# fumiama/Retrieval-based-Voice-Conversion-WebUI

Measured on AMD Instinct MI355X. Metric: real-time factor (audio-sec/wall-sec), 48 kHz v2, 10 s clips, retrieval + NSF-HiFi-GAN decode, higher is better.
Workload: dtype fp16 MFMA operands + fp16 inter-stage streams (ResBlock outputs, ups output of stages 1-3), fp32 accumulate / in-block residual; fp32 MFMA prefilter + fp64 verified IVF distances; 1 GPU; BASELINE configs[1]: v2/48k, 1 x 10 s clip(s) per GPU, T=1198 frames, 599 queries/clip, IVF 10000x768 nlist=256 nprobe=1 k=8 index_rate=0.75; hipgraph=True, index_blob_bytes=32376576, launcher=single process

## Files before the change

retrieval-based-voice-conversion-webui_amd/csrc/ivf.hip:

```cpp
#include <algorithm>
#include <atomic>
#include <cfloat>
#include <cmath>
#include <cstdio>
#include <memory>
#include <string>
#include <vector>

#include "common.hpp"
#include "ivf_format.hpp"
#include "ivf_kmeans.hpp"
#include "ivf_kernels.hpp"
#include "ivf_lm_kernels.hpp"
#include "ivf_add_kernels.hpp"

using namespace rvcmi;

struct rvcmi_ivf {
    int device = 0;
    BlobHeader hdr;
    char* blob = nullptr;
    bool owns_blob = false;
    int64_t cap_nq = 0;
    int cap_nprobe = 0;
// ... 137 lines not shown
    float* feats;
    float rate, omr;
};
static bool search(rvcmi_ivf* h, int64_t nq, const float* q, int k, float* D, int64_t* I, hipStream_t st,
                   const BlendFuse* bf = nullptr) {
    if (!h || nq < 0 || (nq && (!q || !D || !I))) RVCMI_FAIL(RVCMI_ERR_INVALID, "null argument");
    if (k < 1 || k > KMAX)
        RVCMI_FAIL(RVCMI_ERR_INVALID, "k=%d outside [1,%d]: the kernels keep at most %d neighbours per query (RVC asks for 8, "
                   "pipeline.py:126; legacy top-1 tools/cmd/infer-pm-index256.py:161)", k, KMAX, KMAX);
    if (nq == 0) return false;
    DeviceGuard dg(h->device);
    reserve(h, nq);
    const BlobHeader& b = h->hdr;
    const int d = b.d;
    const int np = (int)std::min<int64_t>(b.nprobe, b.nlist);
    HIP_CHECK(hipMemsetAsync(h->flag.p, 0, 4, st));
    const double cflops = 3.0 * (double)nq * b.nlist * d;
    if (np == 1 && !h->opt.on("IVF_COARSE_F64")) {
        h->prof.launch("ivf_coarse", 2.0 * (double)nq * b.nlist * d, (double)nq * d * 4 + (double)b.nlist * d * 4 + 2.0 * nq * b.nlist * 4, st, [&] {
            if (h->cap_chunk <= 0 || !h->cscore.p) RVCMI_FAIL(RVCMI_ERR_INVALID, "coarse score scratch not reserved");
            for (int64_t qs = 0; qs < nq; qs += h->cap_chunk) {
                const int64_t nqc = std::min<int64_t>(h->cap_chunk, nq - qs);
                const int64_t big_blocks = ((b.nlist + 127) / 128) * ((nqc + 63) / 64);
                if (big_blocks >= 512) {
                    dim3 grid((unsigned)((b.nlist + 127) / 128), (unsigned)((nqc + 63) / 64));
                    hipLaunchKernelGGL((k_coarse_gemm<2, 4>), grid, dim3(256), 0, st, q + qs * d, h->centroids(), h->cnorm(), nqc,
                                       b.nlist, d, h->cscore.as<float>());
                } else {
                    dim3 grid((unsigned)((b.nlist + 31) / 32), (unsigned)((nqc + 31) / 32));
                    hipLaunchKernelGGL(k_coarse_gemm_ks, grid, dim3(256), 0, st, q + qs * d, h->centroids(), h->cnorm(), nqc,
                                       b.nlist, d, h->cscore.as<float>());
                }
                hipLaunchKernelGGL(k_coarse_pick, dim3((unsigned)((nqc + 3) / 4)), dim3(256), 0, st, q + qs * d, h->centroids(),
                                   h->cscore.as<float>(), nqc, b.nlist, d, b.cmax, h->assign.as<int64_t>() + qs);
            }
        });
    } else if (np == 1) {
        const size_t smem = align_up((size_t)QT * d * 4, 16) + 4 * QT * 16;
        h->prof.launch("ivf_coarse", cflops, (double)nq * d * 4 + (double)b.nlist * d * 4, st, [&] {
            hipLaunchKernelGGL(k_coarse1, dim3((unsigned)((nq + QT - 1) / QT)), dim3(256), smem, st, q, h->centroids_t(), nq,
                               b.nlist, d, h->assign.as<int64_t>());
        });
    } else {
        h->prof.launch("ivf_coarse", cflops, (double)nq * b.nlist * 8, st, [&] {
            const int64_t tot = nq * b.nlist;
            hipLaunchKernelGGL(k_coarse_dist, dim3((unsigned)((tot + 255) / 256)), dim3(256), 0, st, q, h->centroids(), nq,
                               b.nlist, d, h->cdist.as<double>());
            hipLaunchKernelGGL(k_coarse_select, dim3((unsigned)nq), dim3(64), 0, st, h->cdist.as<double>(), b.nlist, np,
                               h->assign.as<int64_t>());
        });
    }
    const bool lm_wanted = h->opt.geti("IVF_LM", 1) && !h->opt.on("IVF_GENERIC");
    if (lm_wanted && nq >= 64 && !h->lm_warned) {
        const char* why = lm_unusable_reason(h, nq);
        if (why) {
            h->lm_warned = true;
            fprintf(stderr, "[rvcmi] ivf search: %lld queries run on the query-major scan (every probed list is re-read per query) because the "
                    "list-major kernels do not take this call: %s.  Printed once per index.\n", (long long)nq, why);
        }
    }
    if (lm_wanted && lm_usable(h, nq) && h->lm_S.p && nq <= h->lm_cap_nq && h->lm_buf_nq > 0) {
        const int pitch = (int)align_up((uint64_t)h->lm_maxlen, 32);
// ... 452 lines not shown
```

retrieval-based-voice-conversion-webui_amd/csrc/ivf_kernels.hpp:

```cpp
#pragma once
#include <hip/hip_runtime.h>

#include <cfloat>
#include <cmath>
#include <cstdint>

#include "glue_kernels.hpp"
#include "ivf_format.hpp"

namespace rvcmi {


constexpr int QT = 4;

__global__ void __launch_bounds__(256) k_coarse1(const float* __restrict__ q, const float4* __restrict__ cent_t,
                                                 int64_t nq, int64_t nlist, int d, int64_t* __restrict__ assign) {
    extern __shared__ __attribute__((aligned(16))) char smem_raw[];
    float* qs = (float*)smem_raw;
    double* bd = (double*)(smem_raw + align_up((size_t)QT * d * 4, 16));
    int64_t* bi = (int64_t*)(bd + 4 * QT);
    const int64_t q0 = (int64_t)blockIdx.x * QT;
    const int nqb = (int)min((int64_t)QT, nq - q0);
    for (int i = threadIdx.x; i < QT * d; i += 256) {
        int qi = i / d;
        qs[i] = qi < nqb ? q[(q0 + qi) * d + (i - qi * d)] : 0.f;
    }
    __syncthreads();
    double best[QT];
    int64_t besti[QT];
#pragma unroll
    for (int k = 0; k < QT; ++k) { best[k] = INFINITY; besti[k] = INT64_MAX; }
    const int d4 = d >> 2;
// ... 39 lines not shown
        int64_t biv = bi[k];
        for (int w = 1; w < 4; ++w) {
            double od = bd[w * QT + k];
            int64_t oi = bi[w * QT + k];
            if (od < bdv || (od == bdv && oi < biv)) { bdv = od; biv = oi; }
        }
        assign[q0 + k] = biv;
    }
}

constexpr int CG_K = 32, CG_S = 33;
using f32x16 = __attribute__((ext_vector_type(16))) float;
template <int MQ, int NWC>
__global__ void __launch_bounds__(64 * NWC) k_coarse_gemm(const float* __restrict__ q, const float* __restrict__ cent,
                                                          const float* __restrict__ cn, int64_t nq, int64_t nlist, int d,
                                                          float* __restrict__ S) {
    constexpr int NT = 64 * NWC, QR = 32 * MQ, CR = 32 * NWC;
    __shared__ float Qs[QR * CG_S];
    __shared__ float Cs[CR * CG_S];
    const int64_t q0 = (int64_t)blockIdx.y * QR, c0 = (int64_t)blockIdx.x * CR;
    const int wave = threadIdx.x >> 6, lane = threadIdx.x & 63;
    f32x16 acc[MQ];
#pragma unroll
    for (int m = 0; m < MQ; ++m)
#pragma unroll
        for (int e = 0; e < 16; ++e) acc[m][e] = 0.f;
    constexpr int SLOTS = (QR + CR) * (CG_K / 4);
    static_assert(SLOTS % NT == 0, "staging slots must divide evenly");
    constexpr int PER = SLOTS / NT;
    float4 pre[PER];
    auto fetch = [&](int k0) {
#pragma unroll
// ... 62 lines not shown
            float* dst = st + (idx >> 3) * CG_S + (idx & 7) * 4;
            const float4 v = pre[c % D][s2];
            dst[0] = v.x; dst[1] = v.y; dst[2] = v.z; dst[3] = v.w;
        }
        if (c + D < NCH) {
#pragma unroll
            for (int s2 = 0; s2 < 8; ++s2) pre[c % D][s2] = *(const float4*)(src[s2] + kw + (c + D) * kstep + coff);
        }
#pragma unroll
        for (int ks = 0; ks < CG_K / 2; ++ks) acc = __builtin_amdgcn_mfma_f32_32x32x2f32(qa[2 * ks], cb[2 * ks], acc, 0, 0, 0);
    }
}

__global__ void __launch_bounds__(256) k_coarse_gemm_ks(const float* __restrict__ q, const float* __restrict__ cent,
                                                        const float* __restrict__ cn, int64_t nq, int64_t nlist, int d,
                                                        float* __restrict__ S) {
    __shared__ float St[4][64 * CG_S];
    __shared__ float Red[3][64 * 16];
    const int64_t q0 = (int64_t)blockIdx.y * 32, c0 = (int64_t)blockIdx.x * 32;
    const int wave = threadIdx.x >> 6, lane = threadIdx.x & 63;
    float* st = St[wave];
    f32x16 acc;
#pragma unroll
    for (int e = 0; e < 16; ++e) acc[e] = 0.f;
    float4 pre[8];
    auto fetch = [&](int k0) {
#pragma unroll
        for (int it = 0; it < 8; ++it) {
            const int idx = lane + it * 64;
            const int row = idx >> 3, c4 = idx & 7;
            const int kk = min(k0 + c4 * 4, d - 4);
// ... 116 lines not shown
                a0 = fma(t0, t0, a0);
                a1 = fma(t1, t1, a1);
            }
            for (int off = 32; off >= 1; off >>= 1) {
                a0 += __shfl_xor(a0, off, 64);
                a1 += __shfl_xor(a1, off, 64);
            }
            if (a0 < best || (a0 == best && c0 + b0 < besti)) { best = a0; besti = c0 + b0; }
            if (two && (a1 < best || (a1 == best && c0 + b1 < besti))) { best = a1; besti = c0 + b1; }
        }
    }
    if (lane == 0) assign[qi] = besti;
}

__global__ void __launch_bounds__(256) k_coarse_dist(const float* __restrict__ q, const float* __restrict__ cent,
                                                     int64_t nq, int64_t nlist, int d, double* __restrict__ dist) {
    const int64_t i = (int64_t)blockIdx.x * 256 + threadIdx.x;
    if (i >= nq * nlist) return;
    const int64_t qi = i / nlist, c = i - qi * nlist;
    const float* a = q + qi * d;
    const float* b = cent + c * d;
    double acc = 0.0;
    for (int e = 0; e < d; ++e) {
        double t = (double)a[e] - (double)b[e];
        acc = fma(t, t, acc);
    }
    dist[i] = acc;
}
__global__ void __launch_bounds__(64) k_coarse_select(double* __restrict__ dist, int64_t nlist, int nprobe,
                                                      int64_t* __restrict__ assign) {
    const int64_t qi = blockIdx.x;
// ... 413 lines not shown
```

retrieval-based-voice-conversion-webui_amd/csrc/nsf.hip:

```cpp
#include <algorithm>
#include <atomic>
#include <cmath>
#include <functional>
#include <memory>
#include <string>
#include <unordered_map>

#include "common.hpp"
#include "nsf_kernels.hpp"
#include "conv_pack.hpp"
#include "rb_stream.hpp"

namespace rvcmi {

struct Geom {
    int MI, NJ, WCO, TT;
};
static Geom conv_geom(int cout) {
    Geom g;
    g.NJ = 4;
    if (cout >= 256) { g.MI = 2; g.WCO = 4; }
    else if (cout >= 128) { g.MI = 2; g.WCO = 2; }
    else if (cout >= 64) { g.MI = 2; g.WCO = 1; }
    else { g.MI = 1; g.WCO = 1; }
// ... 28 lines not shown
    float lin_w = 1.f, lin_b = 0.f;
    std::vector<Stage> stages;
    DevBuf post_w;
    int c_last = 0;
    size_t S = 0;
    DevBuf P, X0, Ya[RVCMI_MAX_RB], Yb[RVCMI_MAX_RB], H, NZ, har, har2, x2, phase, condv, dbg;
    size_t ws_bytes = 0;
    Profiler prof;
    rvcmi::Options opt;
};

namespace rvcmi {


static void set_lds_limits();
constexpr int RB_KG = 4;
#ifndef RB256_NJ
#define RB256_NJ 4
#endif
static int rb_rows(int C) { return C == 256 ? 32 * RB256_NJ : RB_ROWS; }
constexpr int RB_SPLIT_MAX_ROWS = 1024;
constexpr int RB_SPLIT_MAX_ROWS_128 = 4096;

static void build_stage(Stage& s, const rvcmi_nsf_config* cfg, const WeightMap& wm, int i) {
    const int op = cfg->operand, C0 = cfg->upsample_initial_channel;
    s.cin = C0 >> i;
    s.cout = C0 >> (i + 1);
    s.u = cfg->upsample_rates[i];
    s.k = cfg->upsample_kernel_sizes[i];
    s.pad = (s.k - s.u) / 2;
// ... 83 lines not shown
}

static void nsf_create(const rvcmi_nsf_config* cfg, const rvcmi_tensor* weights, int n_weights, int device, int max_B,
                       int max_T, rvcmi_nsf** out) {
    if (!cfg || !out || (!weights && n_weights)) RVCMI_FAIL(RVCMI_ERR_INVALID, "null argument");
    if (cfg->n_ups < 1 || cfg->n_ups > RVCMI_MAX_UPS || cfg->n_resblock_kernels < 1 ||
        cfg->n_resblock_kernels > RVCMI_MAX_RB)
        RVCMI_FAIL(RVCMI_ERR_INVALID, "bad stage counts");
    if (cfg->operand < 0 || cfg->operand > 2) RVCMI_FAIL(RVCMI_ERR_INVALID, "bad operand type %d", cfg->operand);
    if (max_B < 1 || max_T < 1) RVCMI_FAIL(RVCMI_ERR_INVALID, "max_B/max_T must be positive");
    HIP_CHECK(hipSetDevice(device));
    set_lds_limits();
    rb_stream_prepare();

    std::unique_ptr<rvcmi_nsf> h(new rvcmi_nsf());
    h->opt.load_env({"RB_STREAM", "NO_RB_SPLIT", "POST_DMA", "POST_DBG", "RBF_PAD_TAP", "RBF32_TALL", "DBG", "Y_F16", "X0_F16", "X0_F16_NOSTREAM"});
    rb_stream_load_env(h->opt);
    h->cfg = *cfg;
    h->device = device;
    h->max_B = max_B;
    h->max_T = max_T;
    const int op = cfg->operand;
    WeightMap wm;
    for (int i = 0; i < n_weights; ++i) wm.m[weights[i].name] = &weights[i];

    const int C0 = cfg->upsample_initial_channel, inter = cfg->inter_channels;
    h->C0 = C0;
    {
        const rvcmi_tensor& w = wm.get("conv_pre.weight", {C0, inter, 7});
        const rvcmi_tensor& b = wm.get("conv_pre.bias", {C0});
        const float* wd = w.data;
// ... 32 lines not shown
        upload(h->post_w, wt);
    }
    if (h->c_last & 3) RVCMI_FAIL(RVCMI_ERR_INVALID, "last stage channel count %d", h->c_last);

    if (cfg->n_resblock_kernels > 3) RVCMI_FAIL(RVCMI_ERR_INVALID, "more than 3 resblock kernels per stage is unsupported");
    h->S = S * (size_t)max_B;
    const size_t fb = h->S * sizeof(float);
    h->P.alloc((size_t)max_B * max_T * C0 * sizeof(float));
    h->X0.alloc(fb);
    for (int j = 0; j < cfg->n_resblock_kernels; ++j) {
        h->Ya[j].alloc(fb);
        h->Yb[j].alloc(fb);
    }
    if (op == RVCMI_OPERAND_F32) h->H.alloc(fb);
    else h->H.alloc((size_t)3 * std::max(RB_SPLIT_MAX_ROWS * 256, RB_SPLIT_MAX_ROWS_128 * 128) * 2);
    {
        size_t nz = 0;
        long Ls = max_T;
        for (int i = 0; i < cfg->n_ups; ++i) {
            Ls *= cfg->upsample_rates[i];
            if (h->stages[i].nz_mfma) nz = std::max(nz, (size_t)Ls * h->stages[i].cout);
        }
        if (nz) h->NZ.alloc(nz * max_B * sizeof(float));
    }
    const size_t hb = (size_t)max_B * max_T * upp * sizeof(float);
    h->har.alloc(hb);
    h->har2.alloc(hb);
    h->x2.alloc((size_t)max_B * inter * max_T * sizeof(float));
    h->phase.alloc((size_t)max_B * max_T * sizeof(float));
    h->condv.alloc((size_t)max_B * C0 * sizeof(float));
    HIP_CHECK(hipMemset(h->condv.p, 0, h->condv.bytes));
    h->ws_bytes = (size_t)(1 + 2 * cfg->n_resblock_kernels + (op == RVCMI_OPERAND_F32 ? 1 : 0)) * fb + h->P.bytes + 2 * hb + h->x2.bytes + h->phase.bytes + h->condv.bytes;
    *out = h.release();
}


template <typename OpT, int CIN, int MI, int NJ, int WCO>
static void launch_inst(const ConvArgs& a, int B, hipStream_t st) {
    using TL = Tile<CIN>;
    constexpr int TT = (4 / WCO) * NJ * 32;
    const int co_blocks = (a.cout + 32 * MI * WCO - 1) / (32 * MI * WCO);
    dim3 grid((a.Lq + TT - 1) / TT, co_blocks * a.nphase, B);
    const size_t smem = (size_t)a.tile_rows * TL::STRIDE;
    if (smem > 160 * 1024) RVCMI_FAIL(RVCMI_ERR_INVALID, "LDS tile too large: %zu bytes (cin %d)", smem, CIN);
    hipLaunchKernelGGL((k_conv_mfma<OpT, CIN, MI, NJ, WCO>), grid, dim3(256), smem, st, a);
}

// ... 83 lines not shown
static void launch_rb_pair(int op, int C, const RbPairArgs& ra, int tiles, int nj, int B, int rows, hipStream_t st) {
    if (op == RVCMI_OPERAND_BF16) launch_rb_pair_t<__bf16>(C, ra, tiles, nj, B, rows, st);
    else launch_rb_pair_t<_Float16>(C, ra, tiles, nj, B, rows, st);
}
template <typename OpT>
static void set_lds_rb() {
#define RB_ATTR(C_, MI_, NW_)                                                                                   \
    HIP_CHECK(hipFuncSetAttribute(reinterpret_cast<const void*>(&k_rb_pair<OpT, C_, MI_, NW_, RB_KG>),           \
                                  hipFuncAttributeMaxDynamicSharedMemorySize, 160 * 1024));
    HIP_CHECK(hipFuncSetAttribute(reinterpret_cast<const void*>(&k_rb_pair<OpT, 256, 2, 4, RB_KG, RB256_NJ>),
                                  hipFuncAttributeMaxDynamicSharedMemorySize, 160 * 1024));
    RB_ATTR(128, 2, 2) RB_ATTR(64, 2, 1) RB_ATTR(32, 1, 1) RB_ATTR(16, 1, 1)
#undef RB_ATTR
}

template <typename OpT, int CIN, int MI, int WV>
static void launch_ups_inst(UpsArgs a, int nj, int B, hipStream_t st) {
    const int TQ = 32 * nj * (4 / WV);
    size_t smem = (size_t)a.tile_rows * Tile<CIN>::STRIDE + (a.nz_k1 ? (size_t)(TQ * a.u * a.ns + 16) * 2 : 0);
    if (a.bias_off && a.cout % 4 == 0 && (smem + 15) / 16 * 16 + (size_t)2 * a.cout * 4 <= 160 * 1024) {
        smem = (smem + 15) / 16 * 16;
        a.bias_off = (int)smem;
        smem += (size_t)2 * a.cout * 4;
    } else {
        a.bias_off = 0;
    }
    if (smem > 160 * 1024) RVCMI_FAIL(RVCMI_ERR_INVALID, "upsampler LDS tile too large (%zu B)", smem);
    const int per_block = WV * a.vpw;
    dim3 grid((a.Lin + TQ - 1) / TQ, (a.nvt + per_block - 1) / per_block, B);
    {
        const int esz = a.out_half ? 2 : 4;
        const size_t ot = (size_t)TQ * a.u * ((size_t)a.cout * esz + 16);
        smem = (smem + 15) / 16 * 16;
        if (a.out_tr && grid.y == 1 && (a.cout * esz) % 16 == 0 && smem + ot <= 52 * 1024) {
            a.out_tr_off = (int)smem;
            smem += ot;
        } else {
            a.out_tr = 0;
        }
    }
    if (a.out_tw_off && !a.out_tr && a.out_half && nj == 1 && MI == 2 && a.cout % 64 == 0) {
        smem = (smem + 15) / 16 * 16;
        a.out_tw_off = (int)smem;
        smem += (size_t)4 * 32 * (MI * 64 + 16);
    } else {
        a.out_tw_off = 0;
    }
    if (nj == 4) hipLaunchKernelGGL((k_ups<OpT, CIN, MI, WV, 4>), grid, dim3(256), smem, st, a);
    else if (nj == 2) hipLaunchKernelGGL((k_ups<OpT, CIN, MI, WV, 2>), grid, dim3(256), smem, st, a);
    else hipLaunchKernelGGL((k_ups<OpT, CIN, MI, WV, 1>), grid, dim3(256), smem, st, a);
}
#define RVCMI_UPS_CASES(X, OpT) \
    X(OpT, 512, 2) X(OpT, 256, 2) X(OpT, 128, 2) X(OpT, 64, 1) X(OpT, 32, 1)
template <typename OpT>
static void launch_ups_t(const UpsArgs& a, int wv, int nj, int B, hipStream_t st) {
#define X(OpT_, CIN_, MI_)                                                        \
    if (a.cin == CIN_) {                                                          \
        if (wv == 4) return launch_ups_inst<OpT_, CIN_, MI_, 4>(a, nj, B, st);    \
        if (wv == 2) return launch_ups_inst<OpT_, CIN_, MI_, 2>(a, nj, B, st);    \
        return launch_ups_inst<OpT_, CIN_, MI_, 1>(a, nj, B, st);                 \
    }
    RVCMI_UPS_CASES(X, OpT)
#undef X
    RVCMI_FAIL(RVCMI_ERR_INVALID, "unsupported upsampler C_in %d", a.cin);
}
template <typename OpT>
static void set_lds_ups() {
#define Y(OpT_, CIN_, MI_, WV_, NJ_)                                                                                    \
    HIP_CHECK(hipFuncSetAttribute(reinterpret_cast<const void*>(&k_ups<OpT_, CIN_, MI_, WV_, NJ_>),                      \
                                  hipFuncAttributeMaxDynamicSharedMemorySize, 160 * 1024));
#define X(OpT_, CIN_, MI_)                                                                                              \
    Y(OpT_, CIN_, MI_, 4, 4) Y(OpT_, CIN_, MI_, 4, 2) Y(OpT_, CIN_, MI_, 4, 1) Y(OpT_, CIN_, MI_, 2, 4) Y(OpT_, CIN_, MI_, 2, 2)   \
    Y(OpT_, CIN_, MI_, 2, 1) Y(OpT_, CIN_, MI_, 1, 4) Y(OpT_, CIN_, MI_, 1, 2) Y(OpT_, CIN_, MI_, 1, 1)
    RVCMI_UPS_CASES(X, OpT)
#undef Y
#undef X
}

#ifndef RBF32_NJ
#define RBF32_NJ 3
#define RBF32_OCC 2
#endif
template <int C> struct RbFullGeom;
#ifndef RBF64_NWV
#define RBF64_NWV 8
#endif
#if RBF64_NWV == 8
template <> struct RbFullGeom<64> { static constexpr int MI = 2, NJ = 2, KG = 4, OCC = 2, NWV = 8; };
#else
template <> struct RbFullGeom<64> { static constexpr int MI = 2, NJ = 3, KG = 4, OCC = 1, NWV = 4; };
#endif
// ... 509 lines not shown
        ua.ph_w_off[r] = U.pack_off[r];
        ua.ph_in_off[r] = U.in_off[r];
        lo = std::min(lo, U.in_off[r] - (U.ntaps_p - 1));
        hi = std::max(hi, U.in_off[r]);
    }
    ua.ntaps_p = U.ntaps_p;
    ua.u = s.u;
    ua.cout = C;
    ua.lo = lo;
    ua.bias = U.bias.as<float>();
    ua.out = h->X0.as<float>();
    ua.out_half = p.x0_half ? 1 : 0;
    ua.out_tr = 1;
    ua.out_tw_off = 1;
    ua.out_bstride = L * C;
    if (h->cfg.use_f0 && s.nz_mfma) {
        ConvArgs na = base_args();
        na.in = f.har;
        na.in_bstride = (long)f.Te * upp;
        na.Lin = f.Te * upp;
        na.in_mode = IN_HAR;
        na.hs = s.ns;
        na.hpad = s.npad;
        na.Lq = (int)L;
        na.out_mode = OUT_F32;
        na.out = h->NZ.p;
        na.out_bstride = L * C;
        na.out_C = C;
        na.lens = f.lens;
        na.lmul_in = upp;
        na.lmul_q = lm;
// ... 2 lines not shown
        ua.addend = h->NZ.as<float>();
    } else if (h->cfg.use_f0) {
        ua.nz_k1 = s.nz_k1 ? 1 : 0;
        ua.wnz = s.nz_k1_w.p;
        ua.har = f.har;
        ua.Lh = f.Te * upp;
        ua.Wn = s.noise_w.as<float>();
        ua.bn = s.noise_b.as<float>();
        ua.nk = s.nk;
        ua.ns = s.ns;
        ua.npad = s.npad;
    }
    const int MIu = C >= 64 ? 2 : 1;
    ua.cog = (C + 32 * MIu - 1) / (32 * MIu);
    ua.nvt = s.u * ua.cog;
    const int wv = ua.nvt >= 4 ? 4 : (ua.nvt >= 2 ? 2 : 1);
    int nj = 4;
    const long blocks4 = (long)((Lin + 128 * (4 / wv) - 1) / (128 * (4 / wv))) * B;
    if (blocks4 < 2048 && s.cin >= 128) nj = s.cin >= 512 ? 2 : 1;
    else if (blocks4 < 2048 && s.cin == 64) nj = 2;
    else if (s.cin >= 512) nj = 2;
    else if (s.cin == 128) nj = 1;
    else if (s.cin == 64) nj = 2;
    const int TQ = 32 * nj * (4 / wv);
    ua.tile_rows = TQ + (hi - lo);
    const long qtiles = (Lin + TQ - 1) / TQ;
    int vpw = (ua.nvt + wv - 1) / wv;
    while (vpw > 1 && qtiles * B * ((ua.nvt + wv * vpw - 1) / (wv * vpw)) < 300) --vpw;
    ua.vpw = vpw;
    snprintf(nm, sizeof(nm), "ups_c%d", s.cin);
    const double flops = U.flops_per_pos * (double)Lin * B + 2.0 * s.nk * (double)L * C * B;
    const double bytes = (double)B * Lin * x.C * (x.half ? 2 : 4) * (x.y[1] ? (x.y[2] ? 3 : 2) : 1) + (double)B * L * C * (p.x0_half ? 2 : 4);
    h->prof.launch(nm, flops, bytes, f.st, [&] {
        if (f.op == RVCMI_OPERAND_BF16) launch_ups_t<__bf16>(ua, wv, nj, B, f.st);
        else launch_ups_t<_Float16>(ua, wv, nj, B, f.st);
    });
    HIP_CHECK(hipGetLastError());
}
// ... 295 lines not shown
    return guarded([&] {
        if (!what || !out_host || !shape_out) RVCMI_FAIL(RVCMI_ERR_INVALID, "null argument");
        TapRequest tr;
        tr.what = what;
        tr.out_host = out_host;
        tr.capacity = capacity_floats;
        tr.shape = shape_out;
        nsf_forward(h, B, T, nullptr, x, f0, g, noise, n_res, nullptr, (hipStream_t)stream, &tr);
        if (!tr.done) RVCMI_FAIL(RVCMI_ERR_INVALID, "tap '%s' was not produced", what);
    });
}

int rvcmi_nsf_set_option(rvcmi_nsf* h, const char* key, double value) {
    return guarded([&] {
        if (!h || !key) RVCMI_FAIL(RVCMI_ERR_INVALID, "null argument");
        if ((!strcmp(key, "RBF_PAD_TAP") || !strcmp(key, "RBF32_TALL")) && value == value && value != 0.0 && value != 1.0)
            RVCMI_FAIL(RVCMI_ERR_INVALID, "option '%s' takes 0 or 1", key);
        if (!h->opt.set(key, value)) RVCMI_FAIL(RVCMI_ERR_INVALID, "unknown option '%s' for this handle", key);
    });
}
int rvcmi_nsf_profile_enable(rvcmi_nsf* h, int enable) {
    return guarded([&] {
        if (!h) RVCMI_FAIL(RVCMI_ERR_INVALID, "null handle");
        h->prof.enabled = enable != 0;
    });
}
int rvcmi_nsf_profile_read(rvcmi_nsf* h, rvcmi_kernel_stat* stats, int capacity, int* n, int reset) {
    return guarded([&] {
        if (!h) RVCMI_FAIL(RVCMI_ERR_INVALID, "null handle");
        h->prof.read(stats, capacity, n, reset);
    });
}

// ... 2 lines not shown
```

retrieval-based-voice-conversion-webui_amd/csrc/nsf_kernels.hpp:

```cpp
#pragma once
#include <hip/hip_runtime.h>

#include "exact_fp.hpp"
#include <stdint.h>

namespace rvcmi {

using bf16x8 = __attribute__((ext_vector_type(8))) __bf16;
using f16x8 = __attribute__((ext_vector_type(8))) _Float16;
using f32x16 = __attribute__((ext_vector_type(16))) float;
using f32x4 = __attribute__((ext_vector_type(4))) float;

__device__ __forceinline__ float lrelu(float v, float slope) { return v > 0.f ? v : v * slope; }

__device__ __forceinline__ int item_rows(const int* __restrict__ lens, int b, int mul, int Lmax) {
    return lens ? max(min(Lmax, lens[b] * mul), min(Lmax, mul)) : Lmax;
}


static __global__ void __launch_bounds__(256) k_phase_scan(const float* __restrict__ f0, float* __restrict__ phase,
                                                   int T, float sr, float upp, const int* __restrict__ lens) {
#pragma clang fp contract(off)
    __shared__ double wsum[4];
    const int b = blockIdx.x;
// ... 1321 lines not shown
    int out_tr;
    int out_tr_off;
    int out_tw_off;
    long out_bstride;
    const float* addend;
    const float* har;
    int Lh;
    int Lh_stride;
    const int* lens;
    int lmul, lhmul;
    const float* Wn;
    const float* bn;
    int nk, ns, npad;
    const void* wnz;
    int nz_k1;
    int nvt, cog, vpw;
    int dbg;
    int bias_off;
};

template <typename OpT, int CIN, int MI, int WV, int NJ = 4>
#ifndef UPS_OCC
#define UPS_OCC 2
#endif
static __global__ void __launch_bounds__(256, UPS_OCC) k_ups(UpsArgs a) {
    using TL = Tile<CIN>;
    using frag = typename Op<OpT>::frag;
    constexpr int STRIDE = TL::STRIDE;
    constexpr int C8 = CIN / 8;
    constexpr int WT = 4 / WV;
    constexpr int TQ = 32 * NJ * WT;
    constexpr int SB = 5;
    extern __shared__ __attribute__((aligned(16))) char smem[];
    const int b = blockIdx.z;
    const int q0 = blockIdx.x * TQ;
    const int Linb = item_rows(a.lens, b, a.lmul, a.Lin), Lhb = item_rows(a.lens, b, a.lhmul, a.Lh);
// ... 153 lines not shown
#pragma unroll
        for (int j = 0; j < 2; ++j)
            if ((int)threadIdx.x + 256 * j < hspan) har16[threadIdx.x + 256 * j] = to_op<OpT>(hpre[j]);
        for (int i = threadIdx.x + 512; i < hspan; i += 256) {
            const long idx = hbase + i;
            har16[i] = (idx >= 0 && idx < Lhb) ? to_op<OpT>(hp[idx]) : (OpT)0.f;
        }
    }
    __syncthreads();

    const int wave = threadIdx.x >> 6;
    const int lane = threadIdx.x & 63;
    const int wv = wave % WV, wt = wave / WV;
    const int tw0 = wt * NJ * 32;
    const char* lds_lane = smem + (size_t)(tw0 + (lane & 31)) * STRIDE + (lane >> 5) * 16;
    const float* har = (a.har && !a.nz_k1) ? a.har + (size_t)b * a.Lh_stride : nullptr;
    float* out = a.out + (size_t)b * a.out_bstride;

    for (int i = 0; i < a.vpw; ++i) {
        const int vt = ((int)blockIdx.y * WV + wv) * a.vpw + i;
        if (vt >= a.nvt) break;
        const int r = vt / a.cog;
        const int ct0 = (vt - r * a.cog) * MI;
        f32x16 acc[MI][NJ];
#pragma unroll
        for (int mi = 0; mi < MI; ++mi)
#pragma unroll
            for (int jt = 0; jt < NJ; ++jt)
#pragma unroll
                for (int e = 0; e < 16; ++e) acc[mi][jt][e] = 0.f;
        const OpT* wlane = (const OpT*)a.w + a.ph_w_off[r] + (size_t)ct0 * a.ct_stride + lane * 8;
// ... 11 lines not shown
                for (int e = 0; e < 4; ++e) cv.u[e] = wp[e];
                Bn[jt] = cv.f;
            }
#pragma unroll
            for (int mi = 0; mi < MI; ++mi)
#pragma unroll
                for (int jt = 0; jt < NJ; ++jt) acc[mi][jt] = Op<OpT>::mfma(An[mi], Bn[jt], acc[mi][jt]);
        }

        const float* addend = a.addend ? a.addend + (size_t)b * a.out_bstride : nullptr;
#pragma unroll
        for (int jt = 0; jt < NJ; ++jt) {
            const int q = q0 + tw0 + jt * 32 + (lane & 31);
            const bool valid = q < Linb;
            const int t = min(q, Linb - 1) * a.u + r;
            f32x4 nv[MI][4];
#pragma unroll
            for (int mi = 0; mi < MI; ++mi)
#pragma unroll
                for (int g = 0; g < 4; ++g) {
                    const int co = min((ct0 + mi) * 32 + 8 * g + 4 * (lane >> 5), a.cout - 4);
                    nv[mi][g] = addend ? *(const f32x4*)(addend + (size_t)t * a.cout + co) : f32x4{0.f, 0.f, 0.f, 0.f};
                }
            if (har && !(a.dbg & 4)) {
                const int hb = t * a.ns - a.npad;
                for (int j = 0; j < a.nk; ++j) {
                    const int hi = hb + j;
                    const float hv = (hi >= 0 && hi < Lhb) ? har[hi] : 0.f;
#pragma unroll
                    for (int mi = 0; mi < MI; ++mi)
#pragma unroll
                        for (int g = 0; g < 4; ++g) {
                            const int co = min((ct0 + mi) * 32 + 8 * g + 4 * (lane >> 5), a.cout - 4);
                            const f32x4 wv4 = *(const f32x4*)(a.Wn + (size_t)j * a.cout + co);
                            nv[mi][g] += wv4 * hv;
                        }
                }
            }
            if (valid && !(a.dbg & 16)) {
#pragma unroll
                for (int mi = 0; mi < MI; ++mi)
#pragma unroll
                    for (int g = 0; g < 4; ++g) {
                        const int co = (ct0 + mi) * 32 + 8 * g + 4 * (lane >> 5);
                        if (co >= a.cout) continue;
                        f32x4 v = {acc[mi][jt][4 * g + 0], acc[mi][jt][4 * g + 1], acc[mi][jt][4 * g + 2], acc[mi][jt][4 * g + 3]};
                        const float* bsrc = a.bias_off ? bias_l : a.bias;
                        const float* bnsrc = a.bias_off ? bias_l + a.cout : a.bn;
                        v += *(const f32x4*)(bsrc + co);
                        if (har) v += nv[mi][g] + *(const f32x4*)(bnsrc + co);
                        else if (addend) v += nv[mi][g];
                        else if (a.nz_k1) v += *(const f32x4*)(bnsrc + co);
                        if (a.out_tr) {
                            const int orow = (tw0 + jt * 32 + (lane & 31)) * a.u + r;
                            char* ot = smem + a.out_tr_off;
                            if (a.out_half) *(uint2*)(ot + (size_t)orow * (a.cout * 2 + 16) + co * 2) = pack4_h(v[0], v[1], v[2], v[3]);
                            else *(f32x4*)(ot + (size_t)orow * (a.cout * 4 + 16) + co * 4) = v;
                        } else if (NJ == 1 && a.out_tw_off) {
                            *(uint2*)(smem + a.out_tw_off + (wave * 32 + (lane & 31)) * (MI * 64 + 16) + (mi * 32 + 8 * g + 4 * (lane >> 5)) * 2) =
                                pack4_h(v[0], v[1], v[2], v[3]);
                        } else if (a.out_half) *(uint2*)((_Float16*)a.out + (size_t)b * a.out_bstride + (size_t)t * a.cout + co) = pack4_h(v[0], v[1], v[2], v[3]);
                        else *(f32x4*)(out + (size_t)t * a.cout + co) = v;
                    }
            }
        }
        if (NJ == 1 && a.out_tw_off && !(a.dbg & 16)) {
// ... 391 lines not shown
```

Measured before the change: 5781 x real-time (audio-sec/wall-sec), whole job.

## Fold NSF noise conv into upsampler MFMA epilogue and drop IVF flag memset

For upsampler stages with C_in >= 128 and four channel waves, the harmonic-source noise convolution is now computed as extra MFMAs inside the k_ups kernel rather than as a separate conv writing an fp32 NZ buffer that is read back as an addend. This removes one kernel launch per stage plus the full-resolution NZ write and read, and the NZ workspace is only allocated if some stage cannot fold. The trade-off is extra accumulator registers and weight/harmonic loads in the upsampler, with possible spills or lower occupancy. Separately, the per-search hipMemsetAsync of the IVF flag is replaced by having the first coarse kernel's first thread clear it, saving one graph node.

New measurement: 5773 x real-time (audio-sec/wall-sec), whole job. Within noise of the previous version (-0.1%).

```diff
diff --git a/retrieval-based-voice-conversion-webui_amd/csrc/ivf.hip b/retrieval-based-voice-conversion-webui_amd/csrc/ivf.hip
--- a/retrieval-based-voice-conversion-webui_amd/csrc/ivf.hip
+++ b/retrieval-based-voice-conversion-webui_amd/csrc/ivf.hip
@@ -175,7 +175,7 @@
     const BlobHeader& b = h->hdr;
     const int d = b.d;
     const int np = (int)std::min<int64_t>(b.nprobe, b.nlist);
-    HIP_CHECK(hipMemsetAsync(h->flag.p, 0, 4, st));
+    int* const flag0 = h->flag.as<int>();
     const double cflops = 3.0 * (double)nq * b.nlist * d;
     if (np == 1 && !h->opt.on("IVF_COARSE_F64")) {
         h->prof.launch("ivf_coarse", 2.0 * (double)nq * b.nlist * d, (double)nq * d * 4 + (double)b.nlist * d * 4 + 2.0 * nq * b.nlist * 4, st, [&] {
@@ -186,11 +186,11 @@
                 if (big_blocks >= 512) {
                     dim3 grid((unsigned)((b.nlist + 127) / 128), (unsigned)((nqc + 63) / 64));
                     hipLaunchKernelGGL((k_coarse_gemm<2, 4>), grid, dim3(256), 0, st, q + qs * d, h->centroids(), h->cnorm(), nqc,
-                                       b.nlist, d, h->cscore.as<float>());
+                                       b.nlist, d, h->cscore.as<float>(), qs == 0 ? flag0 : nullptr);
                 } else {
                     dim3 grid((unsigned)((b.nlist + 31) / 32), (unsigned)((nqc + 31) / 32));
                     hipLaunchKernelGGL(k_coarse_gemm_ks, grid, dim3(256), 0, st, q + qs * d, h->centroids(), h->cnorm(), nqc,
-                                       b.nlist, d, h->cscore.as<float>());
+                                       b.nlist, d, h->cscore.as<float>(), qs == 0 ? flag0 : nullptr);
                 }
                 hipLaunchKernelGGL(k_coarse_pick, dim3((unsigned)((nqc + 3) / 4)), dim3(256), 0, st, q + qs * d, h->centroids(),
                                    h->cscore.as<float>(), nqc, b.nlist, d, b.cmax, h->assign.as<int64_t>() + qs);
@@ -200,13 +200,13 @@
         const size_t smem = align_up((size_t)QT * d * 4, 16) + 4 * QT * 16;
         h->prof.launch("ivf_coarse", cflops, (double)nq * d * 4 + (double)b.nlist * d * 4, st, [&] {
             hipLaunchKernelGGL(k_coarse1, dim3((unsigned)((nq + QT - 1) / QT)), dim3(256), smem, st, q, h->centroids_t(), nq,
-                               b.nlist, d, h->assign.as<int64_t>());
+                               b.nlist, d, h->assign.as<int64_t>(), flag0);
         });
     } else {
         h->prof.launch("ivf_coarse", cflops, (double)nq * b.nlist * 8, st, [&] {
             const int64_t tot = nq * b.nlist;
             hipLaunchKernelGGL(k_coarse_dist, dim3((unsigned)((tot + 255) / 256)), dim3(256), 0, st, q, h->centroids(), nq,
-                               b.nlist, d, h->cdist.as<double>());
+                               b.nlist, d, h->cdist.as<double>(), flag0);
             hipLaunchKernelGGL(k_coarse_select, dim3((unsigned)nq), dim3(64), 0, st, h->cdist.as<double>(), b.nlist, np,
                                h->assign.as<int64_t>());
         });
diff --git a/retrieval-based-voice-conversion-webui_amd/csrc/ivf_kernels.hpp b/retrieval-based-voice-conversion-webui_amd/csrc/ivf_kernels.hpp
--- a/retrieval-based-voice-conversion-webui_amd/csrc/ivf_kernels.hpp
+++ b/retrieval-based-voice-conversion-webui_amd/csrc/ivf_kernels.hpp
@@ -13,9 +13,15 @@
 
 constexpr int QT = 4;
 
+__device__ __forceinline__ void clear_search_flag(int* flag) {
+    if (flag && threadIdx.x == 0 && blockIdx.x == 0 && blockIdx.y == 0) *flag = 0;
+}
+
 __global__ void __launch_bounds__(256) k_coarse1(const float* __restrict__ q, const float4* __restrict__ cent_t,
-                                                 int64_t nq, int64_t nlist, int d, int64_t* __restrict__ assign) {
+                                                 int64_t nq, int64_t nlist, int d, int64_t* __restrict__ assign,
+                                                 int* clear_flag = nullptr) {
     extern __shared__ __attribute__((aligned(16))) char smem_raw[];
+    clear_search_flag(clear_flag);
     float* qs = (float*)smem_raw;
     double* bd = (double*)(smem_raw + align_up((size_t)QT * d * 4, 16));
     int64_t* bi = (int64_t*)(bd + 4 * QT);
@@ -85,8 +91,9 @@
 template <int MQ, int NWC>
 __global__ void __launch_bounds__(64 * NWC) k_coarse_gemm(const float* __restrict__ q, const float* __restrict__ cent,
                                                           const float* __restrict__ cn, int64_t nq, int64_t nlist, int d,
-                                                          float* __restrict__ S) {
+                                                          float* __restrict__ S, int* clear_flag = nullptr) {
     constexpr int NT = 64 * NWC, QR = 32 * MQ, CR = 32 * NWC;
+    clear_search_flag(clear_flag);
     __shared__ float Qs[QR * CG_S];
     __shared__ float Cs[CR * CG_S];
     const int64_t q0 = (int64_t)blockIdx.y * QR, c0 = (int64_t)blockIdx.x * CR;
@@ -179,7 +186,8 @@
 
 __global__ void __launch_bounds__(256) k_coarse_gemm_ks(const float* __restrict__ q, const float* __restrict__ cent,
                                                         const float* __restrict__ cn, int64_t nq, int64_t nlist, int d,
-                                                        float* __restrict__ S) {
+                                                        float* __restrict__ S, int* clear_flag = nullptr) {
+    clear_search_flag(clear_flag);
     __shared__ float St[4][64 * CG_S];
     __shared__ float Red[3][64 * 16];
     const int64_t q0 = (int64_t)blockIdx.y * 32, c0 = (int64_t)blockIdx.x * 32;
@@ -326,7 +334,9 @@
 }
 
 __global__ void __launch_bounds__(256) k_coarse_dist(const float* __restrict__ q, const float* __restrict__ cent,
-                                                     int64_t nq, int64_t nlist, int d, double* __restrict__ dist) {
+                                                     int64_t nq, int64_t nlist, int d, double* __restrict__ dist,
+                                                     int* clear_flag = nullptr) {
+    clear_search_flag(clear_flag);
     const int64_t i = (int64_t)blockIdx.x * 256 + threadIdx.x;
     if (i >= nq * nlist) return;
     const int64_t qi = i / nlist, c = i - qi * nlist;
diff --git a/retrieval-based-voice-conversion-webui_amd/csrc/nsf.hip b/retrieval-based-voice-conversion-webui_amd/csrc/nsf.hip
--- a/retrieval-based-voice-conversion-webui_amd/csrc/nsf.hip
+++ b/retrieval-based-voice-conversion-webui_amd/csrc/nsf.hip
@@ -66,6 +66,38 @@
 
 
 static void set_lds_limits();
+
+static bool nz_fold(const rvcmi_nsf* h) { return h->opt.geti("NZ_FOLD", 1) != 0; }
+static int ups_geom(const Stage& s, long Lin, int B, int* wv_out) {
+    const int MIu = s.cout >= 64 ? 2 : 1;
+    const int nvt = s.u * ((s.cout + 32 * MIu - 1) / (32 * MIu));
+    const int wv = nvt >= 4 ? 4 : (nvt >= 2 ? 2 : 1);
+    *wv_out = wv;
+    int nj = 4;
+    const long blocks4 = (long)((Lin + 128 * (4 / wv) - 1) / (128 * (4 / wv))) * B;
+    if (blocks4 < 2048 && s.cin >= 128) nj = s.cin >= 512 ? 2 : 1;
+    else if (blocks4 < 2048 && s.cin == 64) nj = 2;
+    else if (s.cin >= 512) nj = 2;
+    else if (s.cin == 128) nj = 1;
+    else if (s.cin == 64) nj = 2;
+    return nj;
+}
+static bool stage_folds(const Stage& s, long Lin, int B) {
+    int wv = 0;
+    return s.nz_mfma && s.cin >= 128 && ups_geom(s, Lin, B, &wv) != 4 && wv == 4;
+}
+static void reserve_nz(rvcmi_nsf* h) {
+    if (h->NZ.p) return;
+    size_t nz = 0;
+    long Ls = h->max_T;
+    for (int i = 0; i < h->cfg.n_ups; ++i) {
+        Ls *= h->cfg.upsample_rates[i];
+        if (h->stages[i].nz_mfma) nz = std::max(nz, (size_t)Ls * h->stages[i].cout);
+    }
+    if (!nz) return;
+    h->NZ.alloc(nz * h->max_B * sizeof(float));
+    h->ws_bytes += h->NZ.bytes;
+}
 constexpr int RB_KG = 4;
 #ifndef RB256_NJ
 #define RB256_NJ 4
@@ -179,7 +211,7 @@
     rb_stream_prepare();
 
     std::unique_ptr<rvcmi_nsf> h(new rvcmi_nsf());
-    h->opt.load_env({"RB_STREAM", "NO_RB_SPLIT", "POST_DMA", "POST_DBG", "RBF_PAD_TAP", "RBF32_TALL", "DBG", "Y_F16", "X0_F16", "X0_F16_NOSTREAM"});
+    h->opt.load_env({"RB_STREAM", "NO_RB_SPLIT", "POST_DMA", "POST_DBG", "RBF_PAD_TAP", "RBF32_TALL", "DBG", "Y_F16", "X0_F16", "X0_F16_NOSTREAM", "NZ_FOLD"});
     rb_stream_load_env(h->opt);
     h->cfg = *cfg;
     h->device = device;
@@ -242,15 +274,6 @@
     }
     if (op == RVCMI_OPERAND_F32) h->H.alloc(fb);
     else h->H.alloc((size_t)3 * std::max(RB_SPLIT_MAX_ROWS * 256, RB_SPLIT_MAX_ROWS_128 * 128) * 2);
-    {
-        size_t nz = 0;
-        long Ls = max_T;
-        for (int i = 0; i < cfg->n_ups; ++i) {
-            Ls *= cfg->upsample_rates[i];
-            if (h->stages[i].nz_mfma) nz = std::max(nz, (size_t)Ls * h->stages[i].cout);
-        }
-        if (nz) h->NZ.alloc(nz * max_B * sizeof(float));
-    }
     const size_t hb = (size_t)max_B * max_T * upp * sizeof(float);
     h->har.alloc(hb);
     h->har2.alloc(hb);
@@ -259,6 +282,13 @@
     h->condv.alloc((size_t)max_B * C0 * sizeof(float));
     HIP_CHECK(hipMemset(h->condv.p, 0, h->condv.bytes));
     h->ws_bytes = (size_t)(1 + 2 * cfg->n_resblock_kernels + (op == RVCMI_OPERAND_F32 ? 1 : 0)) * fb + h->P.bytes + 2 * hb + h->x2.bytes + h->phase.bytes + h->condv.bytes;
+    bool all_fold = nz_fold(h.get());
+    long Lin = max_T;
+    for (const Stage& s : h->stages) {
+        all_fold = all_fold && (!s.nz_mfma || stage_folds(s, Lin, max_B));
+        Lin *= s.u;
+    }
+    if (!all_fold) reserve_nz(h.get());
     *out = h.release();
 }
 
@@ -372,8 +402,9 @@
 #undef RB_ATTR
 }
 
-template <typename OpT, int CIN, int MI, int WV>
+template <typename OpT, int CIN, int MI, int WV, bool NZF = false>
 static void launch_ups_inst(UpsArgs a, int nj, int B, hipStream_t st) {
+    if (NZF && nj == 4) RVCMI_FAIL(RVCMI_ERR_INVALID, "no folded noise conv for 128-row upsampler tiles");
     const int TQ = 32 * nj * (4 / WV);
     size_t smem = (size_t)a.tile_rows * Tile<CIN>::STRIDE + (a.nz_k1 ? (size_t)(TQ * a.u * a.ns + 16) * 2 : 0);
     if (a.bias_off && a.cout % 4 == 0 && (smem + 15) / 16 * 16 + (size_t)2 * a.cout * 4 <= 160 * 1024) {
@@ -404,16 +435,20 @@
     } else {
         a.out_tw_off = 0;
     }
-    if (nj == 4) hipLaunchKernelGGL((k_ups<OpT, CIN, MI, WV, 4>), grid, dim3(256), smem, st, a);
-    else if (nj == 2) hipLaunchKernelGGL((k_ups<OpT, CIN, MI, WV, 2>), grid, dim3(256), smem, st, a);
-    else hipLaunchKernelGGL((k_ups<OpT, CIN, MI, WV, 1>), grid, dim3(256), smem, st, a);
-}
+    if (nj == 4) hipLaunchKernelGGL((k_ups<OpT, CIN, MI, WV, 4, false>), grid, dim3(256), smem, st, a);
+    else if (nj == 2) hipLaunchKernelGGL((k_ups<OpT, CIN, MI, WV, 2, NZF>), grid, dim3(256), smem, st, a);
+    else hipLaunchKernelGGL((k_ups<OpT, CIN, MI, WV, 1, NZF>), grid, dim3(256), smem, st, a);
+}
+constexpr bool ups_folds(int cin, int wv) { return cin >= 128 && wv == 4; }
 #define RVCMI_UPS_CASES(X, OpT) \
     X(OpT, 512, 2) X(OpT, 256, 2) X(OpT, 128, 2) X(OpT, 64, 1) X(OpT, 32, 1)
 template <typename OpT>
 static void launch_ups_t(const UpsArgs& a, int wv, int nj, int B, hipStream_t st) {
 #define X(OpT_, CIN_, MI_)                                                        \
     if (a.cin == CIN_) {                                                          \
+        if constexpr (ups_folds(CIN_, 4))                                         \
+            if (a.nz_fold && wv == 4) return launch_ups_inst<OpT_, CIN_, MI_, 4, true>(a, nj, B, st); \
+        if (a.nz_fold) RVCMI_FAIL(RVCMI_ERR_INVALID, "no folded noise conv for upsampler C_in %d with %d channel waves", a.cin, wv); \
         if (wv == 4) return launch_ups_inst<OpT_, CIN_, MI_, 4>(a, nj, B, st);    \
         if (wv == 2) return launch_ups_inst<OpT_, CIN_, MI_, 2>(a, nj, B, st);    \
         return launch_ups_inst<OpT_, CIN_, MI_, 1>(a, nj, B, st);                 \
@@ -433,6 +468,11 @@
     RVCMI_UPS_CASES(X, OpT)
 #undef Y
 #undef X
+#define Y(CIN_, NJ_)                                                                                                    \
+    HIP_CHECK(hipFuncSetAttribute(reinterpret_cast<const void*>(&k_ups<OpT, CIN_, 2, 4, NJ_, true>),                     \
+                                  hipFuncAttributeMaxDynamicSharedMemorySize, 160 * 1024));
+    Y(512, 2) Y(512, 1) Y(256, 2) Y(256, 1) Y(128, 2) Y(128, 1)
+#undef Y
 }
 
 #ifndef RBF32_NJ
@@ -972,7 +1012,20 @@
     ua.out_tr = 1;
     ua.out_tw_off = 1;
     ua.out_bstride = L * C;
-    if (h->cfg.use_f0 && s.nz_mfma) {
+    int wv = 0;
+    const int nj = ups_geom(s, Lin, B, &wv);
+    if (h->cfg.use_f0 && s.nz_mfma && nz_fold(h) && stage_folds(s, Lin, B)) {
+        ua.nz_fold = 1;
+        ua.wnf = s.nz.w_pack.p;
+        ua.nf_ct_stride = s.nz.ct_stride;
+        ua.nf_cc = s.nz.cin / 16;
+        ua.har = f.har;
+        ua.Lh = f.Te * upp;
+        ua.bn = s.noise_b.as<float>();
+        ua.ns = s.ns;
+        ua.npad = s.npad;
+    } else if (h->cfg.use_f0 && s.nz_mfma) {
+        if (!h->NZ.p) RVCMI_FAIL(RVCMI_ERR_INVALID, "the unfolded noise conv has no workspace");
         ConvArgs na = base_args();
         na.in = f.har;
         na.in_bstride = (long)f.Te * upp;
@@ -1005,14 +1058,6 @@
     const int MIu = C >= 64 ? 2 : 1;
     ua.cog = (C + 32 * MIu - 1) / (32 * MIu);
     ua.nvt = s.u * ua.cog;
-    const int wv = ua.nvt >= 4 ? 4 : (ua.nvt >= 2 ? 2 : 1);
-    int nj = 4;
-    const long blocks4 = (long)((Lin + 128 * (4 / wv) - 1) / (128 * (4 / wv))) * B;
-    if (blocks4 < 2048 && s.cin >= 128) nj = s.cin >= 512 ? 2 : 1;
-    else if (blocks4 < 2048 && s.cin == 64) nj = 2;
-    else if (s.cin >= 512) nj = 2;
-    else if (s.cin == 128) nj = 1;
-    else if (s.cin == 64) nj = 2;
     const int TQ = 32 * nj * (4 / wv);
     ua.tile_rows = TQ + (hi - lo);
     const long qtiles = (Lin + TQ - 1) / TQ;
@@ -1338,9 +1383,13 @@
 int rvcmi_nsf_set_option(rvcmi_nsf* h, const char* key, double value) {
     return guarded([&] {
         if (!h || !key) RVCMI_FAIL(RVCMI_ERR_INVALID, "null argument");
-        if ((!strcmp(key, "RBF_PAD_TAP") || !strcmp(key, "RBF32_TALL")) && value == value && value != 0.0 && value != 1.0)
+        if ((!strcmp(key, "RBF_PAD_TAP") || !strcmp(key, "RBF32_TALL") || !strcmp(key, "NZ_FOLD")) && value == value && value != 0.0 && value != 1.0)
             RVCMI_FAIL(RVCMI_ERR_INVALID, "option '%s' takes 0 or 1", key);
         if (!h->opt.set(key, value)) RVCMI_FAIL(RVCMI_ERR_INVALID, "unknown option '%s' for this handle", key);
+        if (!strcmp(key, "NZ_FOLD") && !nz_fold(h)) {
+            HIP_CHECK(hipSetDevice(h->device));
+            reserve_nz(h);
+        }
     });
 }
 int rvcmi_nsf_profile_enable(rvcmi_nsf* h, int enable) {
diff --git a/retrieval-based-voice-conversion-webui_amd/csrc/nsf_kernels.hpp b/retrieval-based-voice-conversion-webui_amd/csrc/nsf_kernels.hpp
--- a/retrieval-based-voice-conversion-webui_amd/csrc/nsf_kernels.hpp
+++ b/retrieval-based-voice-conversion-webui_amd/csrc/nsf_kernels.hpp
@@ -1359,12 +1359,16 @@
     int nk, ns, npad;
     const void* wnz;
     int nz_k1;
+    const void* wnf;
+    long nf_ct_stride;
+    int nf_cc;
+    int nz_fold;
     int nvt, cog, vpw;
     int dbg;
     int bias_off;
 };
 
-template <typename OpT, int CIN, int MI, int WV, int NJ = 4>
+template <typename OpT, int CIN, int MI, int WV, int NJ = 4, bool NZF = false>
 #ifndef UPS_OCC
 #define UPS_OCC 2
 #endif
@@ -1548,7 +1552,9 @@
     const int wv = wave % WV, wt = wave / WV;
     const int tw0 = wt * NJ * 32;
     const char* lds_lane = smem + (size_t)(tw0 + (lane & 31)) * STRIDE + (lane >> 5) * 16;
-    const float* har = (a.har && !a.nz_k1) ? a.har + (size_t)b * a.Lh_stride : nullptr;
+    const float* har = (a.har && !a.nz_k1 && !NZF) ? a.har + (size_t)b * a.Lh_stride : nullptr;
+    const float* harf = NZF ? a.har + (size_t)b * a.Lh_stride : nullptr;
+    const int nf_ccr = (a.ns + 15) >> 4;
     float* out = a.out + (size_t)b * a.out_bstride;
 
     for (int i = 0; i < a.vpw; ++i) {
@@ -1590,6 +1596,53 @@
             const int q = q0 + tw0 + jt * 32 + (lane & 31);
             const bool valid = q < Linb;
             const int t = min(q, Linb - 1) * a.u + r;
+            f32x16 accn[MI];
+            if constexpr (NZF) {
+#pragma unroll
+                for (int mi = 0; mi < MI; ++mi)
+#pragma unroll
+                    for (int e = 0; e < 16; ++e) accn[mi][e] = 0.f;
+            }
+            if constexpr (NZF) {
+                static_assert(NJ <= 2, "the folded noise conv next to 128 accumulator registers spills");
+                constexpr int NF_B = NJ == 2 ? 4 : 1;
+                const OpT* wn = (const OpT*)a.wnf + lane * 8;
+                const int ct_last = (a.cout + 31) / 32 - 1;
+                const long hb0 = (long)t * a.ns - a.npad + 8 * (lane >> 5);
+#pragma clang loop unroll(disable)
+                for (int jb = 0; jb < 2 * (4 / NF_B) && !(a.dbg & 4); ++jb) {
+                    const int j = jb / (4 / NF_B), cc0 = (jb - j * (4 / NF_B)) * NF_B;
+                    if (cc0 >= nf_ccr) continue;
+                    frag Anf[NF_B][MI];
+                    float4 flo[NF_B], fhi[NF_B];
+#pragma unroll
+                    for (int i = 0; i < NF_B; ++i)
+                        if (cc0 + i < nf_ccr) {
+                            const int cc = cc0 + i;
+                            const long base = hb0 + (long)j * a.ns + 16 * cc;
+                            flo[i] = *(const float4*)(harf + min(max(base, 0L), (long)Lhb - 4));
+                            fhi[i] = *(const float4*)(harf + min(max(base + 4, 0L), (long)Lhb - 4));
+#pragma unroll
+                            for (int mi = 0; mi < MI; ++mi)
+                                Anf[i][mi] = *(const frag*)(wn + (size_t)min(ct0 + mi, ct_last) * a.nf_ct_stride + (size_t)(j * a.nf_cc + cc) * 512);
+                        }
+#pragma unroll
+                    for (int i = 0; i < NF_B; ++i)
+                        if (cc0 + i < nf_ccr) {
+                            const int cc = cc0 + i;
+                            const long base = hb0 + (long)j * a.ns + 16 * cc;
+                            const bool inframe = 16 * cc + 8 * (lane >> 5) < a.ns;
+                            const bool oklo = inframe && base >= 0 && base + 4 <= Lhb;
+                            const bool okhi = inframe && base + 4 >= 0 && base + 8 <= Lhb;
+                            const float f[8] = {flo[i].x, flo[i].y, flo[i].z, flo[i].w, fhi[i].x, fhi[i].y, fhi[i].z, fhi[i].w};
+                            frag Bn;
+#pragma unroll
+                            for (int e = 0; e < 8; ++e) Bn[e] = ((e < 4) ? oklo : okhi) ? to_op<OpT>(f[e]) : (OpT)0.f;
+#pragma unroll
+                            for (int mi = 0; mi < MI; ++mi) accn[mi] = Op<OpT>::mfma(Anf[i][mi], Bn, accn[mi]);
+                        }
+                }
+            }
             f32x4 nv[MI][4];
 #pragma unroll
             for (int mi = 0; mi < MI; ++mi)
@@ -1597,6 +1650,10 @@
                 for (int g = 0; g < 4; ++g) {
                     const int co = min((ct0 + mi) * 32 + 8 * g + 4 * (lane >> 5), a.cout - 4);
                     nv[mi][g] = addend ? *(const f32x4*)(addend + (size_t)t * a.cout + co) : f32x4{0.f, 0.f, 0.f, 0.f};
+                    if constexpr (NZF) {
+                        const f32x4 an = {accn[mi][4 * g + 0], accn[mi][4 * g + 1], accn[mi][4 * g + 2], accn[mi][4 * g + 3]};
+                        nv[mi][g] = an + *(const f32x4*)((a.bias_off ? bias_l + a.cout : a.bn) + co);
+                    }
                 }
             if (har && !(a.dbg & 4)) {
                 const int hb = t * a.ns - a.npad;
@@ -1625,7 +1682,7 @@
                         const float* bnsrc = a.bias_off ? bias_l + a.cout : a.bn;
                         v += *(const f32x4*)(bsrc + co);
                         if (har) v += nv[mi][g] + *(const f32x4*)(bnsrc + co);
-                        else if (addend) v += nv[mi][g];
+                        else if (addend || NZF) v += nv[mi][g];
                         else if (a.nz_k1) v += *(const f32x4*)(bnsrc + co);
                         if (a.out_tr) {
                             const int orow = (tw0 + jt * 32 + (lane & 31)) * a.u + r;
```
